# protolambda/go-kzg

Measured on AMD Instinct MI355X. Metric: KZG commitments/sec (CommitToPoly, 4096-element blob); FK20 half: value_fk20_4096, higher is better.
Workload: dtype u32; 1 GPU; CommitToPoly, 4096-coeff blobs, eth/trusted_setup.json monomial setup (s=1337), 4096 blobs/step/GPU resident in HBM, fixed-base table budget 110 GB (library default 110 GB: signed 16-bit windows, 8 of them walked by both GLV halves of every scalar, 103 GB; see table_sweep); global_batch=4096, parallelism=dp1 (independent blobs, no data-path collective)

## Files before the change

go-kzg_amd/__init__.py:

```python
import ctypes as C
import os

import numpy as np

_HERE = os.path.dirname(os.path.abspath(__file__))
LIB_PATH = os.environ.get("KZG_HIP_LIB") or os.path.join(_HERE, "libkzg_hip.so")

OK, ERR_TOO_WIDE, ERR_NOT_POW2, ERR_LEN_MISMATCH, ERR_UPPER_HALF, ERR_BAD_ARG, ERR_BAD_POINT, ERR_NO_DEVICE, ERR_HIP, ERR_UNSUPPORTED, ERR_RECOVERY, ERR_BAD_BLOB = range(12)


class KzgError(Exception):

    def __init__(self, status, msg=""):
        super().__init__("kzg_hip status %d %s" % (status, msg))
        self.status = status


class KzgPanic(KzgError):
    """The reference panics (kzg.go:22-27,44-52,74-91; fk20_single.go:60-62,140-154; bls_kilic.go:133-135)."""


class NoDeviceError(KzgError):
    pass

# ... 32 lines not shown
        "kzg_hip_points_set_table_budget_gb": (i32, [vp, C.c_double]),
        "kzg_hip_lincomb_points": (i32, [vp, vp, u64, vp]), "kzg_hip_lincomb_points_batch": (i32, [vp, vp, u64, u64, vp]),
        "kzg_hip_lincomb_points_batch_dev": (i32, [vp, vp, u64, u64, vp, vp]), "kzg_hip_g1_to_compressed": (i32, [vp, vp, u64, vp]),
        "kzg_hip_g1_from_compressed": (i32, [vp, vp, u64, vp]), "kzg_hip_g1_mul_vec": (i32, [vp, vp, vp, u64, vp]),
        "kzg_hip_generate_testing_setup_g1": (i32, [vp, vp, u64, vp]),
        "kzg_hip_g1_marshal_text": (i32, [vp, vp, u64, vp]), "kzg_hip_g1_unmarshal_text": (i32, [vp, C.c_char_p, u64, vp]),
        "kzg_hip_trusted_setup_from_json": (i32, [vp, C.c_char_p, u64, vp, vp, u64, C.POINTER(u64), C.POINTER(u64)]),
        "kzg_hip_kzg_set_table_budget_gb": (i32, [vp, C.c_double]),
        "kzg_hip_kzg_settings_new": (i32, [vp, vp, u64, pp]), "kzg_hip_kzg_settings_free": (None, [vp]),
        "kzg_hip_commit_to_poly": (i32, [vp, vp, u64, vp]), "kzg_hip_commit_to_poly_batch": (i32, [vp, vp, u64, u64, vp]),
        "kzg_hip_commit_to_poly_batch_dev": (i32, [vp, vp, u64, u64, vp, vp]),
        "kzg_hip_compute_proof_single": (i32, [vp, vp, u64, u64, vp]),
        "kzg_hip_compute_proof_single_batch": (i32, [vp, vp, u64, u64, vp, vp]),
        "kzg_hip_compute_proof_single_batch_dev": (i32, [vp, vp, u64, u64, vp, vp, vp]),
        "kzg_hip_compute_proof_multi": (i32, [vp, vp, u64, u64, u64, vp]),
        "kzg_hip_check_proof_multi_interpolation": (i32, [vp, vp, u64, vp, vp, vp]),
        "kzg_hip_g2_from_compressed": (i32, [vp, vp, u64, vp]), "kzg_hip_pairings_verify_batch": (i32, [vp, vp, vp, vp, vp, u64, vp]),
        "kzg_hip_kzg_set_secret_g2": (i32, [vp, vp, u64]), "kzg_hip_check_proof_single_batch": (i32, [vp, vp, vp, vp, vp, u64, vp]),
        "kzg_hip_check_proof_multi_batch": (i32, [vp, vp, vp, vp, vp, u64, u64, vp]),
        "kzg_hip_eth_set_setup_g2": (i32, [vp, vp, u64]), "kzg_hip_eth_verify_kzg_proof_batch": (i32, [vp, vp, vp, vp, vp, u64, vp]),
        "kzg_hip_pairing_test": (i32, [vp, vp, vp, u64, vp]),
        "kzg_hip_toeplitz_part2": (i32, [vp, vp, vp, u64, vp]), "kzg_hip_toeplitz_part3": (i32, [vp, vp, u64, vp]),
        "kzg_hip_fk20_single_settings_new": (i32, [vp, u64, pp]), "kzg_hip_fk20_single_settings_free": (None, [vp]),
        "kzg_hip_fk20_single_x_ext_fft": (i32, [vp, vp]), "kzg_hip_fk20_single": (i32, [vp, vp, u64, vp]),
        "kzg_hip_fk20_single_batch": (i32, [vp, vp, u64, u64, vp]), "kzg_hip_fk20_single_batch_dev": (i32, [vp, vp, u64, u64, vp, vp]),
        "kzg_hip_fk20_single_da_optimized": (i32, [vp, vp, u64, vp]), "kzg_hip_da_using_fk20": (i32, [vp, vp, u64, vp]),
        "kzg_hip_da_using_fk20_batch": (i32, [vp, vp, u64, u64, vp]), "kzg_hip_da_using_fk20_batch_dev": (i32, [vp, vp, u64, u64, vp, vp]),
        "kzg_hip_fk20_multi_settings_new": (i32, [vp, u64, u64, pp]), "kzg_hip_fk20_multi_settings_free": (None, [vp]),
        "kzg_hip_fk20_multi": (i32, [vp, vp, u64, vp]), "kzg_hip_fk20_multi_da_optimized": (i32, [vp, vp, u64, vp]),
        "kzg_hip_da_using_fk20_multi": (i32, [vp, vp, u64, vp]),
        "kzg_hip_da_using_fk20_multi_batch_dev": (i32, [vp, vp, u64, u64, vp, vp]),
        "kzg_hip_fk20_multi_hext_slice_dev": (i32, [vp, vp, u64, u64, u64, vp, vp]),
        "kzg_hip_fk20_multi_finish_dev": (i32, [vp, vp, i32, vp, vp]),
        "kzg_hip_eth_settings_new": (i32, [vp, vp, u64, pp]), "kzg_hip_eth_settings_free": (None, [vp]),
        "kzg_hip_eth_blob_to_kzg_commitment_batch": (i32, [vp, vp, u64, vp, vp]),
        "kzg_hip_eth_compute_kzg_proof": (i32, [vp, vp, u64, vp, vp, vp]),
        "kzg_hip_eth_compute_kzg_proof_batch": (i32, [vp, vp, u64, u64, vp, vp, vp, vp]),
        "kzg_hip_eth_compute_kzg_proof_batch_dev": (i32, [vp, vp, u64, u64, vp, vp, vp, vp, vp]),
        "kzg_hip_eth_compute_aggregate_kzg_proof": (i32, [vp, vp, u64, vp, vp]),
        "kzg_hip_eth_compute_aggregated_poly_and_commitment": (i32, [vp, vp, vp, u64, vp, vp, vp, vp]),
        "kzg_hip_test_sha256": (None, [vp, u64, vp]),
        "kzg_hip_evaluate_poly_in_evaluation_form": (i32, [vp, vp, u64, vp, u32, vp]),
        "kzg_hip_eth_evaluate_polynomial_in_evaluation_form": (i32, [vp, vp, u64, vp, vp]),
        "kzg_hip_bench_threads_fft_fr": (i32, [vp, vp, u64, u64, u32, u32, vp, C.POINTER(C.c_double)]),
        "kzg_hip_bench_drop_in_eth_proof": (i32, [vp, vp, u64, u64, u32, u32, vp, C.POINTER(C.c_double)]),
        "kzg_hip_zero_poly_via_multiplication": (i32, [vp, vp, u64, u64, vp, vp]),
        "kzg_hip_recover_poly_from_samples": (i32, [vp, vp, vp, u64, vp]),
        "kzg_hip_calibrate": (i32, [vp, C.POINTER(C.c_double), C.POINTER(C.c_double), C.POINTER(C.c_double)]),
        "kzg_hip_bench_drop_in": (i32, [vp, i32, vp, u64, u64, u32, u32, vp, C.POINTER(C.c_double)]),
        "kzg_hip_coalesce_stats": (i32, [vp, i32, C.POINTER(u64)]),
        "kzg_hip_lincomb_promotions": (i32, [vp, C.POINTER(u64), C.POINTER(u64)]),
        "kzg_hip_test_fp_inv": (i32, [vp, vp, u64, vp, vp, C.POINTER(C.c_double), C.POINTER(C.c_double)]),
        "kzg_hip_test_fr_inv": (i32, [vp, vp, u64, vp, vp, vp]),
        "kzg_hip_kzg_table_info": (i32, [vp, C.POINTER(C.c_uint32), C.POINTER(C.c_uint32), C.POINTER(u64)]), "kzg_hip_kzg_table_additions": (u32, [vp]), "kzg_hip_kzg_set_projective_outputs": (i32, [vp, i32]),
        "kzg_hip_da_using_fk20_multi_batch": (i32, [vp, vp, u64, u64, vp]),
        "kzg_hip_multi_settings_new": (i32, [C.POINTER(i32), u32, u32, vp, u64, pp]), "kzg_hip_multi_settings_free": (None, [vp]),
        "kzg_hip_multi_device_count": (u32, [vp]), "kzg_hip_multi_device": (i32, [vp, u32]),
        "kzg_hip_multi_fft": (vp, [vp, u32]), "kzg_hip_multi_kzg": (vp, [vp, u32]),
        "kzg_hip_multi_transport": (C.c_char_p, [vp]), "kzg_hip_multi_transport_note": (C.c_char_p, [vp]), "kzg_hip_multi_transport_check": (C.c_char_p, [vp]), "kzg_hip_multi_exchanges": (u64, [vp]),
        "kzg_hip_multi_set_fft_sharding": (i32, [vp, i32]), "kzg_hip_multi_set_table_budget_gb": (i32, [vp, C.c_double]),
        "kzg_hip_multi_commit_to_poly_batch": (i32, [vp, vp, u64, u64, vp]),
        "kzg_hip_multi_compute_proof_single_batch": (i32, [vp, vp, u64, u64, vp, vp]),
        "kzg_hip_multi_fft_fr_batch": (i32, [vp, vp, u64, u64, i32, vp]), "kzg_hip_multi_das_fft_extension_batch": (i32, [vp, vp, u64, u64]),
        "kzg_hip_multi_eth_settings_new": (i32, [vp, vp, u64, pp]), "kzg_hip_multi_eth_settings_free": (None, [vp]),
        "kzg_hip_multi_eth_blob_to_kzg_commitment_batch": (i32, [vp, vp, u64, vp, vp]),
        "kzg_hip_multi_eth_compute_kzg_proof_batch": (i32, [vp, vp, u64, u64, vp, vp, vp, vp]),
        "kzg_hip_multi_fk20_single_settings_new": (i32, [vp, u64, pp]), "kzg_hip_multi_fk20_single_settings_free": (None, [vp]),
        "kzg_hip_multi_da_using_fk20_batch": (i32, [vp, vp, u64, u64, vp]), "kzg_hip_multi_da_using_fk20": (i32, [vp, vp, u64, vp]),
        "kzg_hip_multi_fk20_multi_settings_new": (i32, [vp, u64, u64, pp]), "kzg_hip_multi_fk20_multi_settings_free": (None, [vp]),
        "kzg_hip_multi_da_using_fk20_multi_batch": (i32, [vp, vp, u64, u64, vp]), "kzg_hip_multi_da_using_fk20_multi": (i32, [vp, vp, u64, vp]),
        "kzg_hip_bench_poly_lincomb_dev": (i32, [vp, vp, u64, vp, u64, u64, vp, vp]),
        "kzg_hip_prof_reset": (None, [vp, i32]), "kzg_hip_prof_read": (i32, [vp, C.c_char_p, C.POINTER(C.c_double), C.POINTER(u64)]),
    }
    for name, (res, args) in sig.items():
        if os.environ.get("KZG_HIP_LIB_ALLOW_MISSING") and not hasattr(L, name):
            continue
        f = getattr(L, name)
        f.restype, f.argtypes = res, args
    _lib = L
    return L


API_SYMBOLS = None


def device_count():
    return lib().kzg_hip_device_count()


class pinned:

    def __init__(self, array):
        self.a = array

    def __enter__(self):
        _chk(lib().kzg_hip_host_register(self.a.ctypes.data, self.a.nbytes))
        return self.a

    def __exit__(self, *exc):
        lib().kzg_hip_host_unregister(self.a.ctypes.data)
        return False


_ERR_STATUS = (ERR_TOO_WIDE, ERR_NOT_POW2)


# ... 760 lines not shown
```

go-kzg_amd/csrc/capi_bench.hip:

```cpp
#include "capi_common.hpp"

namespace {
struct prof_rec { std::string name; hipEvent_t e0, e1; };
std::mutex g_prof_mu;
bool g_prof_on = false;
std::vector<prof_rec> g_prof;
}
namespace kzg {
void prof_begin(hipStream_t s, const char *name) {
    if (!g_prof_on) return;
    std::lock_guard<std::mutex> lk(g_prof_mu);
    prof_rec r; r.name = name;
    hipEventCreate(&r.e0); hipEventCreate(&r.e1);
    hipEventRecord(r.e0, s);
    g_prof.push_back(r);
}
void prof_end(hipStream_t s, const char *name) {
    if (!g_prof_on) return;
    std::lock_guard<std::mutex> lk(g_prof_mu);
    for (size_t i = g_prof.size(); i-- > 0;)
        if (g_prof[i].name == name) { hipEventRecord(g_prof[i].e1, s); break; }
}
}

// ... 130 lines not shown
            hipEventRecord(e1, s); hipEventSynchronize(e1);
            float ms = 0; hipEventElapsedTime(&ms, e0, e1);
            if (rep && ms < best) best = ms;
        }
        return (double)best * 1e-3;
    };
    const double lanes = (double)blocks * threads;
    *mad_per_s = lanes * CAL_ITERS * 8 / timed(0);
    *add_per_s = lanes * CAL_ITERS * 8 / timed(1);
    *fp_mul_per_s = lanes * 64 * 2 / timed(2);
    hipEventDestroy(e0); hipEventDestroy(e1);
    HIPCHK(hipGetLastError());
    return KZG_HIP_OK;
}
int kzg_hip_test_fp_inv(kzg_hip_fft *fs, const void *in_fp, uint64_t n, void *out_coop, void *out_lane, double *ms_coop, double *ms_lane) {
    if (!fs || !in_fp || !n || n > (1u << 20)) return KZG_HIP_ERR_BAD_ARG;
    dev_guard g(fs);
    hipStream_t s = fs->stream;
    dtmp<fp> d_in(s), d_a(s), d_b(s);
    CHK(d_in.alloc(n)); CHK(d_a.alloc(n)); CHK(d_b.alloc(n));
    HIPCHK(hipMemcpyAsync(d_in.p, in_fp, n * sizeof(fp), hipMemcpyHostToDevice, s));
    hipEvent_t e0, e1;
    HIPCHK(hipEventCreate(&e0)); HIPCHK(hipEventCreate(&e1));
    for (int which = 0; which < 2; which++) {
        void *out = which ? out_lane : out_coop; double *ms = which ? ms_lane : ms_coop;
        if (!out) continue;
        hipEventRecord(e0, s);
        launch_fp_inv_both(s, d_in.p, d_a.p, d_b.p, n, which ? 2 : 1);
        hipEventRecord(e1, s);
        HIPCHK(hipMemcpyAsync(out, which ? d_b.p : d_a.p, n * sizeof(fp), hipMemcpyDeviceToHost, s));
        HIPCHK(hipStreamSynchronize(s));
        float t = 0; hipEventElapsedTime(&t, e0, e1);
        if (ms) *ms = t;
    }
    hipEventDestroy(e0); hipEventDestroy(e1);
    HIPCHK(hipGetLastError());
    return KZG_HIP_OK;
}
int kzg_hip_test_fr_inv(kzg_hip_fft *fs, const void *in_fr, uint64_t n, void *out_coop, void *out_lane, void *out_block) {
    if (!fs || !in_fr || !n || n > (1u << 20) || !out_coop || !out_lane || !out_block) return KZG_HIP_ERR_BAD_ARG;
    dev_guard g(fs);
    hipStream_t s = fs->stream;
    dtmp<fr> d_in(s), d_a(s), d_b(s), d_c(s);
    CHK(d_in.alloc(n)); CHK(d_a.alloc(n)); CHK(d_b.alloc(n)); CHK(d_c.alloc(n));
    HIPCHK(hipMemcpyAsync(d_in.p, in_fr, n * sizeof(fr), hipMemcpyHostToDevice, s));
    launch_fr_inv_test(s, d_in.p, n, d_a.p, d_b.p, d_c.p);
    HIPCHK(hipGetLastError());
    HIPCHK(hipMemcpyAsync(out_coop, d_a.p, n * sizeof(fr), hipMemcpyDeviceToHost, s));
    HIPCHK(hipMemcpyAsync(out_lane, d_b.p, n * sizeof(fr), hipMemcpyDeviceToHost, s));
    HIPCHK(hipMemcpyAsync(out_block, d_c.p, n * sizeof(fr), hipMemcpyDeviceToHost, s));
    HIPCHK(hipStreamSynchronize(s));
    return KZG_HIP_OK;
}
int kzg_hip_coalesce_stats(kzg_hip_kzg *ks, int op, uint64_t out[8]) {
    if (!ks || !out || op < 0 || op > 1) return KZG_HIP_ERR_BAD_ARG;
    for (int i = 0; i < 8; i++) out[i] = 0;
    std::lock_guard<std::mutex> lk(ks->fs->mu);
    coalescer *co = op == 0 ? ks->co_commit.get() : ks->co_proof.get();
    if (co) co->stats(out);
    return KZG_HIP_OK;
}
void kzg_hip_prof_reset(kzg_hip_fft *fs, int enable) {
    (void)fs;
    std::lock_guard<std::mutex> lk(g_prof_mu);
    for (auto &r : g_prof) { hipEventDestroy(r.e0); hipEventDestroy(r.e1); }
    g_prof.clear();
    g_prof_on = enable != 0;
}
int kzg_hip_prof_read(kzg_hip_fft *fs, const char *kernel, double *total_ms, uint64_t *launches) {
    if (!fs || !kernel) return KZG_HIP_ERR_BAD_ARG;
    std::lock_guard<std::mutex> lk(g_prof_mu);
    double tot = 0; uint64_t cnt = 0;
    for (auto &r : g_prof) {
        if (r.name != kernel) continue;
        HIPCHK(hipEventSynchronize(r.e1));
        float ms = 0;
        HIPCHK(hipEventElapsedTime(&ms, r.e0, r.e1));
        tot += ms; cnt++;
    }
    if (total_ms) *total_ms = tot;
    if (launches) *launches = cnt;
    return KZG_HIP_OK;
}
```

go-kzg_amd/csrc/capi_kzg.hip:

```cpp
#include "capi_common.hpp"

int kzg_settings_build(kzg_hip_fft *fs, const void *points_g1, uint64_t n, kzg_hip_kzg **out) {
    dev_guard g(fs);
    hipStream_t s = fs->stream;
    std::unique_ptr<kzg_hip_kzg, void (*)(kzg_hip_kzg *)> own(new kzg_hip_kzg, kzg_hip_kzg_settings_free);
    kzg_hip_kzg *ks = own.get();
    ks->fs = fs; ks->n_setup = n;
    dtmp<g1j> d_raw(s);
    CHK(d_raw.alloc(n));
    HIPCHK(hipMalloc((void **)&ks->d_secret, n * sizeof(g1j)));
    HIPCHK(hipMalloc((void **)&ks->d_secret_a, n * sizeof(g1a)));
    HIPCHK(hipMemcpyAsync(d_raw.p, points_g1, n * sizeof(g1j), hipMemcpyHostToDevice, s));
    launch_g1_from_kilic(s, d_raw.p, n);
    launch_g1_normalize(s, d_raw.p, ks->d_secret, n);
    launch_g1_to_affine(s, ks->d_secret, ks->d_secret_a, n);
    HIPCHK(hipGetLastError());
    HIPCHK(hipStreamSynchronize(s));
    *out = own.release();
    return KZG_HIP_OK;
}
int kzg_hip_kzg_settings_new(kzg_hip_fft *fs, const void *secret_g1, uint64_t n_setup, kzg_hip_kzg **out) {
    if (!fs || !out || !secret_g1) return KZG_HIP_ERR_BAD_ARG;
    *out = nullptr;
    if (n_setup < fs->W) return KZG_HIP_ERR_LEN_MISMATCH;
// ... 15 lines not shown
double table_budget_gb(const char *env, double cap_gb, double headroom_gb) {
    if (const char *e = getenv(env)) return atof(e);
    size_t free_b = 0, total_b = 0;
    if (hipMemGetInfo(&free_b, &total_b) != hipSuccess) return 0.0;
    double g = (double)free_b / 1e9 - headroom_gb;
    return g > cap_gb ? cap_gb : (g > 0.0 ? g : 0.0);
}
uint32_t fb_windows(uint32_t c) {
    uint32_t nw = (255 + c - 1) / c, sh = c * (nw - 1);
    uint64_t top = (0x73eda753299d7d48ull >> (sh - 192)) + 1;
    return top > (1ull << (c - 1)) ? nw + 1 : nw;
}

#ifndef FB_DEFAULT_BUDGET_GB
#define FB_DEFAULT_BUDGET_GB 110.0
#endif
uint32_t fb_windows_glv(uint32_t c) { return (128 + c - 1) / c; }
bool fb_glv_enabled() {
    static const bool on = [] { const char *e = getenv("KZG_HIP_FB_GLV"); return !(e && !strcmp(e, "0")); }();
    return on;
}
int ensure_fixed_table(kzg_hip_kzg *ks, hipStream_t) {
    if (ks->d_fixed || ks->fixed_plan.c == 0xffffffffu) return KZG_HIP_OK;
    hipStream_t s = ks->fs->stream;
    double budget_gb = ks->budget_gb >= 0.0 ? ks->budget_gb : table_budget_gb("KZG_HIP_FB_BUDGET_GB", FB_DEFAULT_BUDGET_GB, 24.0);
    if (ks->n_setup < 64) { ks->fixed_plan.c = 0xffffffffu; return KZG_HIP_OK; }
    const bool glv = fb_glv_enabled();
    for (uint32_t c = 16; c >= 5; c--) {
        if (glv ? (c == 14) : (c == 15)) continue;
        const uint32_t nwin = glv ? fb_windows_glv(c) : fb_windows(c);
        double bytes = (double)nwin * (double)ks->n_setup * (double)(1u << (c - 1)) * sizeof(g1a);
        if (bytes > budget_gb * 1e9) continue;
        msm_plan p{};
        p.c = c; p.nwin = nwin; p.nb = 1u << (c - 1); p.ngroups = 1; p.fixed = 1; p.glv = glv ? 1 : 0; p.table_n = ks->n_setup;
        size_t entries = (size_t)p.nwin * ks->n_setup * p.nb;
        g1a *tab = nullptr;
        if (hipMalloc((void **)&tab, entries * sizeof(g1a)) != hipSuccess) { (void)hipGetLastError(); continue; }
        hipError_t e = launch_fb_build(s, ks->d_secret_a, ks->n_setup, p.c, p.nwin, tab);
        if (e == hipSuccess) e = hipStreamSynchronize(s);
        if (e != hipSuccess) { (void)hipGetLastError(); hipFree(tab); continue; }
        ks->d_fixed = tab; ks->fixed_plan = p;
        return KZG_HIP_OK;
    }
    ks->fixed_plan.c = 0xffffffffu;
    return KZG_HIP_OK;
}

int commit_rows(kzg_hip_kzg *ks, hipStream_t s, const fr *d_sc, uint64_t n, uint64_t batch, g1j *d_out, uint64_t sc_stride, bool to_kilic) {
    CHK(ensure_fixed_table(ks, s));
    bool fixed = ks->d_fixed != nullptr;
    if (!sc_stride) sc_stride = n;
    msm_plan p = fixed ? ks->fixed_plan : classic_plan(ks->n_setup);
    if (!fixed && !msm_index_range_ok(p, n)) return KZG_HIP_ERR_TOO_WIDE;
    size_t ws_main = fixed ? fb_partials_bytes(n, batch) : msm_workspace_bytes(p, n, batch);
    dtmp<uint8_t> d_ws(s);
    CHK(d_ws.alloc(ws_main));
    if (fixed) launch_fb_msm(s, ks->d_fixed, p.table_n, p.c, p.nwin, d_sc, sc_stride, n, batch, d_ws.p, d_out, to_kilic, p.glv != 0, to_kilic && ks->projective.load(std::memory_order_relaxed));
    else launch_msm(s, p, ks->d_secret_a, d_sc, sc_stride, n, batch, d_ws.p, d_out, to_kilic);
    HIPCHK(hipGetLastError());
    return KZG_HIP_OK;
}
int kzg_hip_kzg_set_table_budget_gb(kzg_hip_kzg *ks, double gb) {
    if (!ks || !(gb >= 0.0)) return KZG_HIP_ERR_BAD_ARG;
    std::unique_lock<std::shared_mutex> tl(ks->tab_mu);
    dev_guard g(ks->fs);
    if (ks->d_fixed) { HIPCHK(hipDeviceSynchronize()); HIPCHK(hipFree(ks->d_fixed)); ks->d_fixed = nullptr; }
    ks->fixed_plan = msm_plan{};
    ks->budget_gb = gb;
    return KZG_HIP_OK;
}

int kzg_hip_commit_to_poly_batch_dev(kzg_hip_kzg *ks, const void *d_coeffs_fr, uint64_t n, uint64_t batch, void *d_out_g1, void *stream) {
    if (!ks || !d_out_g1) return KZG_HIP_ERR_BAD_ARG;
    if (n > ks->n_setup) return KZG_HIP_ERR_LEN_MISMATCH;
    if (!batch) return KZG_HIP_OK;
    if (n == 0 || !d_coeffs_fr) return KZG_HIP_ERR_BAD_ARG;
    dev_guard g(ks->fs);
    return commit_rows(ks, (hipStream_t)stream, (const fr *)d_coeffs_fr, n, batch, (g1j *)d_out_g1);
}
namespace {
std::mutex g_reg_mu;
std::map<uintptr_t, size_t> g_registered;
}
const void *host_mapped_pointer(const void *host, size_t bytes) {
    hipPointerAttribute_t a;
    if (hipPointerGetAttributes(&a, host) != hipSuccess) { (void)hipGetLastError(); return nullptr; }
    if (a.type != hipMemoryTypeHost || !a.devicePointer) return nullptr;
    const uintptr_t h = (uintptr_t)host;
    {
        std::lock_guard<std::mutex> lk(g_reg_mu);
        auto it = g_registered.upper_bound(h);
        if (it != g_registered.begin()) {
            --it;
            if (h >= it->first && h < it->first + it->second) return (h + bytes <= it->first + it->second) ? a.devicePointer : nullptr;
        }
    }
    hipDeviceptr_t base = nullptr; size_t size = 0;
    if (hipMemGetAddressRange(&base, &size, (hipDeviceptr_t)a.devicePointer) != hipSuccess) { (void)hipGetLastError(); return nullptr; }
    const uintptr_t d = (uintptr_t)a.devicePointer, b = (uintptr_t)base;
    return (d >= b && d + bytes <= b + size) ? a.devicePointer : nullptr;
}
int h2d_copy(void *dst, const void *src, size_t bytes, hipStream_t s) {
    uintptr_t p = (uintptr_t)src; uint8_t *d = (uint8_t *)dst;
    while (bytes) {
        size_t chunk = bytes;
        {
            std::lock_guard<std::mutex> lk(g_reg_mu);
// ... 339 lines not shown
```

go-kzg_amd/csrc/internal.hpp:

```cpp
#pragma once
#include <hip/hip_runtime.h>
#include <stdint.h>
#include "field.hpp"
#include "g1.hpp"

namespace kzg {

void launch_fr_fft(hipStream_t s, const fr *in, uint64_t in_stride, uint64_t n_in, fr *out, uint64_t n, uint64_t batch,
                   const fr *roots, uint64_t W, const fr *scale, const uint32_t *tw4096 = nullptr, const fr *roots_l = nullptr);
void launch_das_ext(hipStream_t s, fr *vals, uint64_t n, uint64_t batch, const fr *expanded, const fr *reversed, uint64_t W,
                    const fr *inv_n, const uint32_t *tw2048 = nullptr);
void launch_toeplitz_coeffs(hipStream_t s, const fr *poly, uint64_t poly_stride, uint64_t n, uint64_t l, uint64_t batch, fr *out,
                            const fr *scale);
void launch_quotient_linear(hipStream_t s, const fr *poly, uint64_t poly_stride, uint64_t n, uint64_t batch, const fr *x, fr *q, uint64_t q_stride);
void launch_fr_from_u64(hipStream_t s, const uint64_t *in, uint64_t in_stride, fr *out, uint64_t n);
void launch_fr_zero_tails(hipStream_t s, fr *rows, uint64_t n_max, uint64_t batch, const uint64_t *lens, uint64_t lens_stride);
void launch_fr_any_nonzero(hipStream_t s, const fr *vals, uint64_t n, uint32_t *flag);
void launch_fr_powers(hipStream_t s, const fr *base, uint64_t n, fr *out);

void launch_fr_from_le32(hipStream_t s, const uint8_t *in, fr *out, uint64_t per_blob, uint64_t batch, uint32_t *bad);
void launch_fr_to_le32(hipStream_t s, const fr *in, uint8_t *out, uint64_t n);
void launch_fr_bitrev_gather(hipStream_t s, const fr *in, fr *out, uint64_t n);
constexpr uint64_t ZERO_TREE_LEAF = 16;
void launch_zero_leaves(hipStream_t s, const fr *expanded, uint64_t stride, const uint64_t *missing, uint64_t n_missing, uint64_t leaves, fr *a);
// ... 5 lines not shown
void launch_eth_quotient(hipStream_t s, const fr *poly, uint64_t poly_stride, const fr *domain, uint64_t n, uint64_t batch, const fr *z, uint64_t z_stride,
                         const fr *inv_n, fr *q, fr *y_out, uint32_t *flag, uint64_t dom_stride = 1, fr *scratch = nullptr);
uint64_t eth_quotient_scratch_elems(uint64_t n, uint64_t batch);

void launch_fr_scale_by_inv_powers(hipStream_t s, fr *c, const fr *x, uint64_t n, fr *xpow_n);

void launch_zero_eval_direct(hipStream_t s, const fr *expanded, uint64_t stride, const uint64_t *missing, uint64_t n_missing, uint64_t length, fr *zero_eval);
void launch_fr_scale_by_powers(hipStream_t s, fr *poly, const fr *base, uint64_t n);
void launch_fr_pointwise(hipStream_t s, const fr *a, const fr *b, const uint8_t *present, fr *out, uint64_t n, int mode, uint32_t *flag);

void launch_g1_mul_vec(hipStream_t s, const g1j *pts, uint64_t pts_mod, const fr *scalars, uint64_t s_stride, uint64_t n, g1j *out);
hipError_t launch_g1_file_msm(hipStream_t s, const g1j *files, const fr *scalars, uint64_t nfiles, uint64_t k2, uint64_t j0, uint64_t cnt,
                              uint64_t batch, g1j *out);
void launch_g1_bitrev_copy(hipStream_t s, const g1j *in, uint64_t in_stride, uint64_t n_valid, g1j *out, uint64_t n, uint64_t batch);
void launch_g1_fft_stage(hipStream_t s, g1j *data, uint64_t n, uint64_t batch, uint64_t m, const fr *roots, const int8_t *wnaf, uint64_t W);
void launch_g1_fft_stage_dif(hipStream_t s, g1j *data, uint64_t n, uint64_t batch, uint64_t m, const fr *roots, const int8_t *wnaf, uint64_t W);
void launch_g1_clear_odd(hipStream_t s, g1j *data, uint64_t n_total);
void launch_g1_take_even(hipStream_t s, const g1j *in, g1j *out, uint64_t total);
bool g1_quad_enabled();
void launch_fb_direct_pass1(hipStream_t s, const g1a *table, uint64_t table_n, uint32_t c, uint32_t nwin, const fr *scalars, const fr *roots, uint64_t W, uint64_t batch,
                            uint32_t logR, g1j *out, bool glv = false);
void launch_g1_stage_coop_dif(hipStream_t s, int lanes, g1j *data, uint64_t n, uint64_t batch, uint64_t m, const fr *roots, const int8_t *wnaf, uint64_t W, uint64_t total);
void launch_g1_stage_coop_dit(hipStream_t s, int lanes, g1j *data, uint64_t n, uint64_t batch, uint64_t m, const fr *roots, const int8_t *wnaf, uint64_t W, uint64_t total);
void launch_g1_direct_coop(hipStream_t s, int lanes, uint32_t wgs, size_t pad_lds, const g1j *src, uint64_t src_stride, uint64_t src_valid, g1j *dst, uint32_t logn, uint32_t logR,
                           uint64_t Ns, const fr *roots, uint64_t W, const fr *sc, uint64_t total, uint32_t logT, uint32_t logU);
void launch_g1_fft_direct(hipStream_t s, const g1j *in, uint64_t in_stride, uint64_t n_valid, g1j *data, g1j *tmp, uint64_t n, uint64_t batch, const fr *roots,
                          uint64_t W, const fr *scale, uint32_t max_logr = 4, int lanes = 1, uint32_t bits_done = 0, uint64_t n_out = 0);
void launch_g1_normalize(hipStream_t s, const g1j *in, g1j *out, uint64_t n, bool to_kilic = false);
void launch_fr_inv_test(hipStream_t s, const fr *in, uint64_t n, fr *out_coop, fr *out_lane, fr *out_block);
void launch_fp_inv_both(hipStream_t s, const fp *in, fp *out_coop, fp *out_lane, uint64_t n, int mode);
void launch_g1_from_kilic(hipStream_t s, g1j *data, uint64_t n);
void launch_g1_to_affine(hipStream_t s, const g1j *in, g1a *out, uint64_t n);
void launch_g1_compress(hipStream_t s, const g1j *in, uint8_t *out48, uint64_t n);
void launch_g1_decompress(hipStream_t s, const uint8_t *in48, g1j *out, uint64_t n, uint32_t *bad_flag);
void launch_g1_fixed_base_powers(hipStream_t s, const fr *powers, uint64_t n, g1j *out);

uint64_t device_simd_lanes();
inline uint64_t device_simds() { return device_simd_lanes() / 64; }
struct msm_plan {
    uint32_t c;
    uint32_t nwin;
    uint32_t nb;
    uint32_t ngroups;
    uint32_t fixed;
    uint32_t glv;
    uint64_t table_n;
};
inline bool msm_index_range_ok(const msm_plan &p, uint64_t n) { return n < (1ull << 27) && 2 * p.table_n < (1ull << 30); }
size_t msm_workspace_bytes(const msm_plan &p, uint64_t n, uint64_t batch);
void launch_msm(hipStream_t s, const msm_plan &p, const g1a *table, const fr *scalars, uint64_t sc_stride, uint64_t n, uint64_t batch, void *workspace, g1j *out,
                bool to_kilic);
void launch_msm_window_table(hipStream_t s, const g1a *pts, uint64_t n, uint32_t c, uint32_t nwin, g1j *tmp, g1a *out);

size_t fb_partials_bytes(uint64_t n, uint64_t batch);
hipError_t launch_fb_build(hipStream_t s, const g1a *pts, uint64_t n, uint32_t c, uint32_t nwin, g1a *table);
void launch_fb_msm(hipStream_t s, const g1a *table, uint64_t table_n, uint32_t c, uint32_t nwin, const fr *scalars, uint64_t sc_stride, uint64_t n,
                   uint64_t batch, void *partials, g1j *out, bool to_kilic, bool glv = false, bool projective = false);

void launch_fb_mul_vec(hipStream_t s, const g1a *table, uint64_t table_n, uint32_t c, uint32_t nwin, const fr *scalars, uint64_t row, uint64_t j0,
                       uint64_t cnt, uint64_t batch, g1j *out, bool glv = false);
void launch_fb_mul_vec_dif2(hipStream_t s, const g1a *table, uint64_t table_n, uint32_t c, uint32_t nwin, const fr *scalars, const fr *roots, uint64_t W,
                            uint64_t batch, g1j *out, bool glv = false);
void launch_fb_mul_vec_files(hipStream_t s, const g1a *table, uint64_t table_n, uint32_t c, uint32_t nwin, const fr *scalars, uint64_t row, uint64_t j0,
                             uint64_t cnt, uint64_t batch, g1j *out, bool glv = false);
void launch_g1_sum_files(hipStream_t s, const g1j *tmp, uint64_t nfiles, uint64_t cnt, uint64_t batch, g1j *out);

struct g2j; struct g2_prepared;
void launch_g2_from_compressed(hipStream_t s, const uint8_t *in96, g2j *out_kilic, uint64_t n, uint32_t *bad_flag);
void launch_g2_prepare(hipStream_t s, const g2j *in_kilic, uint64_t n, g2_prepared *out);
void launch_pairs_g1_from_kilic(hipStream_t s, const g1j *a1, const g1j *b1, uint64_t n, g1j *p0, g1j *p1);
void launch_kzg_check_inputs(hipStream_t s, const g1j *c, const g1j *pi, const fr *ys, const g1j *es, const fr *bs, uint64_t n, g1j *p0, g1j *p1);
void launch_fr_rows_scale_by_inv_powers(hipStream_t s, fr *c, uint64_t np, const fr *xs, uint64_t count, fr *xpow_n);
void launch_eth_check_inputs(hipStream_t s, const uint8_t *c48, const uint8_t *zs, const uint8_t *ys, const uint8_t *pi48, uint64_t n, g1j *p0, g1j *p1, uint8_t *status);
void launch_pairing_check(hipStream_t s, bool shared_lines, const g2_prepared *q0, const g2_prepared *q1, const g1j *p0, const g1j *p1, uint64_t n, uint8_t *ok);
void launch_pairing_value(hipStream_t s, const g1j *g1_kilic, const g2_prepared *q, uint64_t n, fp *out);

void prof_begin(hipStream_t s, const char *name);
void prof_end(hipStream_t s, const char *name);

}
```

go-kzg_amd/csrc/k_msm.hip:

```cpp
#include "internal.hpp"
#include "g1_quad.hpp"
#include "coop_inv.hpp"
#include <atomic>
#include <cstring>

namespace kzg {

#define MSM_SORT_T 1024
#define MSM_ACC_BLOCK 128
#define MSM_NB 128

struct fb_partial { uint32_t w[52]; uint32_t inf; };
__device__ __forceinline__ void fb_partial_store(fb_partial &o, const g1x_acc &a) {
#pragma unroll
    for (int i = 0; i < 13; i++) { o.w[i] = a.v.x.l[i]; o.w[13 + i] = a.v.y.l[i]; o.w[26 + i] = a.v.zz.l[i]; o.w[39 + i] = a.v.zzz.l[i]; }
    o.inf = a.inf ? 1u : 0u;
}
__device__ __forceinline__ void fb_partial_load(const fb_partial &p, g1xq &v) {
#pragma unroll
    for (int i = 0; i < 13; i++) { v.x.l[i] = p.w[i]; v.y.l[i] = p.w[13 + i]; v.zz.l[i] = p.w[26 + i]; v.zzz.l[i] = p.w[39 + i]; }
}

template <uint32_t DELTA, bool ROW> __device__ __forceinline__ uint32_t lane_down(uint32_t v) {
    if constexpr (ROW && DELTA < 16) return (uint32_t)__builtin_amdgcn_update_dpp((int)v, (int)v, 0x100 + DELTA, 0xf, 0xf, false);
// ... 728 lines not shown
        if (in_phi && !phi) { if (!acc.inf) acc.v.x = mulq(acc.v.x, unpackq(glv_beta())); in_phi = false; }
        uint32_t m[4], sgn;
        if (keep_ok && !phi) {
            const uint32_t at = slot < FB_KEEP ? slot : 0; slot++;
#pragma unroll
            for (int j = 0; j < 4; j++) m[j] = kept[at][j];
            sgn = kept[at][4];
            if (slot == (uint32_t)(nvh / L)) slot = 0;
        } else {
            const glv_halves h = glv_split_signed(from_mont<FrP>(sc[i]));
#pragma unroll
            for (int j = 0; j < 4; j++) m[j] = phi ? h.k2[j] : h.k1[j];
            sgn = phi ? h.neg2 : h.neg1;
            if (keep_ok) {
                const uint32_t at = slot < FB_KEEP ? slot : 0; slot++;
#pragma unroll
                for (int j = 0; j < 4; j++) kept[at][j] = h.k1[j];
                kept[at][4] = h.neg1;
                if (slot == (uint32_t)(nvh / L)) slot = 0;
            }
        }
        uint32_t raw, carry = 0, mag, ng;
        if (SPLIT) {
#pragma nounroll
            for (uint32_t w = 0; w < w0; w++) carry = (mag_bits(m, w * c, c) + carry > D) ? 1u : 0u;
        }
        raw = mag_bits(m, w0 * c, c) + carry;
        if (raw > D) { carry = 1; mag = (1u << c) - raw; ng = 1; } else { carry = 0; mag = raw; ng = 0; }
        g1a qn = table[((uint64_t)w0 * table_n + i) * D + (mag ? mag - 1 : 0)];
#pragma nounroll
        for (uint32_t w = w0; w < w1; w++) {
            g1a q = qn;
            const uint32_t cmag = mag, cng = ng;
            if (w + 1 < w1) {
                raw = mag_bits(m, (w + 1) * c, c) + carry;
                if (raw > D) { carry = 1; mag = (1u << c) - raw; ng = 1; } else { carry = 0; mag = raw; ng = 0; }
                qn = table[((uint64_t)(w + 1) * table_n + i) * D + (mag ? mag - 1 : 0)];
            }
            if (cmag) {
                if (cng ^ sgn) q.y = neg<FpP>(q.y);
                acc.add(q);
                in_phi = phi;
            }
        }
    }
    if (in_phi && !acc.inf) acc.v.x = mulq(acc.v.x, unpackq(glv_beta()));
#ifdef KZG_REDUCE_WAVE_COOP
    fb_block_reduce_coop(acc, buf, &lds, tid);
#else
    fb_block_reduce_quad(acc, buf, tid);
#endif
    if (tid == 0) fb_partial_store(partials[blockIdx.x], acc);
}
__global__ __launch_bounds__(256) void k_fb_finish(const fb_partial *partials, uint32_t blocks_per_blob, uint64_t batch, g1j *out, int to_kilic) {
    __shared__ fb_partial buf[64];
    const uint64_t b = blockIdx.x;
#ifdef KZG_REDUCE_WAVE_COOP
    __shared__ coop_lds lds;
    coop_ctx c; c.L = &lds; c.wave = threadIdx.x >> 6; c.col = threadIdx.x & 63u; c.set = 0;
    const uint32_t col = c.col;
    g1x_acc acc; acc.init();
    acc.v = g1xq_from_affine(g1a_inf());
    const uint32_t rounds = (blocks_per_blob + 63) / 64;
#pragma nounroll
    for (uint32_t r = 0; r < rounds; r++) {
        const uint32_t j = r * 64 + col;
        const bool have = j < blocks_per_blob;
        const fb_partial &pj = partials[b * blocks_per_blob + (have ? j : 0)];
        g1xq w; fb_partial_load(pj, w);
        coop_acc_add(acc, w, !have || pj.inf != 0, c);
    }
    const uint32_t live = blocks_per_blob < 64 ? blocks_per_blob : 64;
    uint32_t off = 1;
    while (off < live) off *= 2;
#pragma nounroll
    for (off >>= 1; off >= 1; off >>= 1) {
        const bool have = col < off && col + off < live;
        g1xq w; uint32_t wi;
        point_down_any(w, wi, acc.v, acc.inf ? 1u : 0u, off);
        coop_acc_add(acc, w, !have || wi != 0, c);
    }
    const bool first_wave = c.wave == 0;
#else
    const uint32_t tid = threadIdx.x, role = tid & 3u, quad = tid >> 2, col = tid & 63u;
#ifdef KZG_FINISH_TIMING
    const uint64_t tf0 = wall_clock64();
#endif
    g1x_acc acc; acc.init();
    acc.v = g1xq_from_affine(g1a_inf());
    const uint32_t rounds = (blocks_per_blob + 63) / 64;
    g1xq wn; bool wn_inf;
    { const bool have = quad < blocks_per_blob; const fb_partial &pj = partials[b * blocks_per_blob + (have ? quad : 0)]; fb_partial_load(pj, wn); wn_inf = !have || pj.inf != 0; }
#pragma nounroll
    for (uint32_t r = 0; r < rounds; r++) {
        const g1xq w = wn; const bool winf = wn_inf;
        if (r + 1 < rounds) {
            const uint32_t j = (r + 1) * 64 + quad;
            const bool have = j < blocks_per_blob;
            const fb_partial &pj = partials[b * blocks_per_blob + (have ? j : 0)];
            fb_partial_load(pj, wn); wn_inf = !have || pj.inf != 0;
        }
        quad_acc_add_nl(acc, w, winf, role);
    }
#ifdef KZG_FINISH_TIMING
    __syncthreads(); const uint64_t tf1 = wall_clock64();
#endif
// ... 228 lines not shown
    out[t] = acc.to_jac();
}
void launch_fb_mul_vec_files(hipStream_t s, const g1a *table, uint64_t table_n, uint32_t c, uint32_t nwin, const fr *scalars, uint64_t row, uint64_t j0,
                             uint64_t cnt, uint64_t batch, g1j *out, bool glv) {
    uint64_t total = batch * cnt;
    if (!total) return;
    prof_begin(s, "fb_mul_vec");
    if (glv) hipLaunchKernelGGL(k_fb_mul_vec_files<true>, dim3((uint32_t)((total + FB_BLOCK - 1) / FB_BLOCK)), dim3(FB_BLOCK), 0, s, table, table_n, c, nwin, 1u << (c - 1), scalars,
                                j0, cnt, row, total, out);
    else hipLaunchKernelGGL(k_fb_mul_vec_files<false>, dim3((uint32_t)((total + FB_BLOCK - 1) / FB_BLOCK)), dim3(FB_BLOCK), 0, s, table, table_n, c, nwin, 1u << (c - 1), scalars,
                            j0, cnt, row, total, out);
    prof_end(s, "fb_mul_vec");
}
void launch_fb_mul_vec(hipStream_t s, const g1a *table, uint64_t table_n, uint32_t c, uint32_t nwin, const fr *scalars, uint64_t row, uint64_t j0,
                       uint64_t cnt, uint64_t batch, g1j *out, bool glv) {
    uint64_t total = batch * (table_n / row) * cnt;
    if (!total) return;
    prof_begin(s, "fb_mul_vec");
    if (glv) hipLaunchKernelGGL(k_fb_mul_vec<true>, dim3((uint32_t)((total + FB_BLOCK - 1) / FB_BLOCK)), dim3(FB_BLOCK), 0, s, table, table_n, c, nwin, 1u << (c - 1), scalars,
                                j0, cnt, row, total, out);
    else hipLaunchKernelGGL(k_fb_mul_vec<false>, dim3((uint32_t)((total + FB_BLOCK - 1) / FB_BLOCK)), dim3(FB_BLOCK), 0, s, table, table_n, c, nwin, 1u << (c - 1), scalars,
                            j0, cnt, row, total, out);
    prof_end(s, "fb_mul_vec");
}

uint64_t device_simd_lanes() {
    static std::atomic<uint64_t> lanes_of_device[64];
    int dev = 0;
    (void)hipGetDevice(&dev);
    std::atomic<uint64_t> &slot = lanes_of_device[dev >= 0 && dev < 64 ? dev : 0];
    uint64_t lanes = slot.load(std::memory_order_relaxed);
    if (!lanes) {
        int cus = 256;
        if (hipDeviceGetAttribute(&cus, hipDeviceAttributeMultiprocessorCount, dev) != hipSuccess) { (void)hipGetLastError(); cus = 256; }
        lanes = (uint64_t)(cus > 0 ? cus : 256) * 4 * 64;
        slot.store(lanes, std::memory_order_relaxed);
    }
    return lanes;
}
static uint32_t fb_blocks_per_blob(uint64_t n, uint64_t batch, uint32_t *wsplit = nullptr) {
    static const uint64_t forced_lanes = [] { const char *e = getenv("KZG_HIP_FB_LANES"); return e ? strtoull(e, nullptr, 10) : 0ull; }();
    uint64_t lanes = forced_lanes ? forced_lanes : 2 * device_simd_lanes();
    if (lanes < FB_ACC_BLOCK) lanes = FB_ACC_BLOCK;
    uint64_t target = lanes / FB_ACC_BLOCK;
    uint64_t bpb = target / (batch ? batch : 1);
    uint32_t split = 1;
    while (split < 8 && (batch ? batch : 1) * n * split * 2 <= lanes) split *= 2;
    if (wsplit) *wsplit = split;
    uint64_t maxb = (n * split + FB_ACC_BLOCK - 1) / FB_ACC_BLOCK;
    if (bpb > maxb) bpb = maxb;
    if (bpb < 1) bpb = 1;
    return (uint32_t)bpb;
}
size_t fb_partials_bytes(uint64_t n, uint64_t batch) { return (((size_t)std::max(fb_blocks_per_blob(n, batch), fb_blocks_per_blob(2 * n, batch)) * batch * sizeof(fb_partial)) + 15) / 16 * 16; }

void launch_fb_msm(hipStream_t s, const g1a *table, uint64_t table_n, uint32_t c, uint32_t nwin, const fr *scalars, uint64_t sc_stride, uint64_t n,
                   uint64_t batch, void *partials, g1j *out, bool to_kilic, bool glv, bool projective) {
    if (!batch) return;
    const int fin = (to_kilic ? 1 : 0) | (projective ? 2 : 0);
    uint32_t split = 1;
    uint32_t bpb = fb_blocks_per_blob(glv ? 2 * n : n, batch, &split);
    if (split > nwin) split = nwin;
    prof_begin(s, "fb_accumulate");
    if (glv) {
        if (split > 1) hipLaunchKernelGGL(k_fb_accumulate_glv<true>, dim3((uint32_t)(batch * bpb)), dim3(FB_ACC_BLOCK), 0, s, table, table_n, c, nwin, 1u << (c - 1), scalars, sc_stride, n,
                                          bpb, split, (fb_partial *)partials);
        else hipLaunchKernelGGL(k_fb_accumulate_glv<false>, dim3((uint32_t)(batch * bpb)), dim3(FB_ACC_BLOCK), 0, s, table, table_n, c, nwin, 1u << (c - 1), scalars, sc_stride, n, bpb,
                                1u, (fb_partial *)partials);
    } else if (split > 1) hipLaunchKernelGGL(k_fb_accumulate<true>, dim3((uint32_t)(batch * bpb)), dim3(FB_ACC_BLOCK), 0, s, table, table_n, c, nwin, 1u << (c - 1), scalars, sc_stride, n,
                                      bpb, split, (fb_partial *)partials);
    else hipLaunchKernelGGL(k_fb_accumulate<false>, dim3((uint32_t)(batch * bpb)), dim3(FB_ACC_BLOCK), 0, s, table, table_n, c, nwin, 1u << (c - 1), scalars, sc_stride, n, bpb,
                            1u, (fb_partial *)partials);
    prof_end(s, "fb_accumulate");
    if (bpb <= FB_FINISH_LANES_MAX) hipLaunchKernelGGL(k_fb_finish_lanes, dim3((uint32_t)((batch + 63) / 64)), dim3(64), 0, s, (const fb_partial *)partials, bpb, batch, out, fin);
    else hipLaunchKernelGGL(k_fb_finish, dim3((uint32_t)batch), dim3(256), 0, s, (const fb_partial *)partials, bpb, batch, out, fin);
}
hipError_t launch_fb_build(hipStream_t s, const g1a *pts, uint64_t n, uint32_t c, uint32_t nwin, g1a *table) {
    uint32_t D = 1u << (c - 1);
    g1j *rows_j = nullptr; g1a *rows = nullptr; fp *ztmp = nullptr, *ptmp = nullptr;
    uint64_t lanes_all = (uint64_t)nwin * n;
    hipError_t e;
    if ((e = hipMallocAsync((void **)&rows_j, lanes_all * sizeof(g1j), s)) != hipSuccess) return e;
    if ((e = hipMallocAsync((void **)&rows, lanes_all * sizeof(g1a), s)) != hipSuccess) { hipFreeAsync(rows_j, s); return e; }
    launch_msm_window_table(s, pts, n, c, nwin, rows_j, rows);
    uint64_t per_win = n * D * sizeof(fp);
    uint32_t slab = (uint32_t)((1ull << 30) / (per_win ? per_win : 1));
    if (slab < 1) slab = 1;
    if (slab > nwin) slab = nwin;
    if ((e = hipMallocAsync((void **)&ztmp, (uint64_t)slab * per_win, s)) != hipSuccess) { hipFreeAsync(rows_j, s); hipFreeAsync(rows, s); return e; }
    if ((e = hipMallocAsync((void **)&ptmp, (uint64_t)slab * per_win, s)) != hipSuccess) { hipFreeAsync(rows_j, s); hipFreeAsync(rows, s); hipFreeAsync(ztmp, s); return e; }
    for (uint32_t w0 = 0; w0 < nwin; w0 += slab) {
        uint32_t ws = (w0 + slab <= nwin) ? slab : nwin - w0;
        uint64_t lanes = (uint64_t)ws * n;
        uint32_t S = D;
        while (S > 64 && lanes * (D / S) < (1ull << 20)) S >>= 1;
        dim3 g((uint32_t)((lanes * (D / S) + FB_BLOCK - 1) / FB_BLOCK)), b(FB_BLOCK);
        hipLaunchKernelGGL(k_fb_build_pass1, g, b, 0, s, rows + (uint64_t)w0 * n, lanes, D, S, table + (uint64_t)w0 * n * D, ztmp);
        hipLaunchKernelGGL(k_fb_build_pass2, g, b, 0, s, lanes, D, S, table + (uint64_t)w0 * n * D, ztmp, ptmp);
    }
    hipFreeAsync(rows_j, s); hipFreeAsync(rows, s); hipFreeAsync(ztmp, s); hipFreeAsync(ptmp, s);
    return hipGetLastError();
}

__global__ __launch_bounds__(MSM_ACC_BLOCK, 2) void k_msm_window_rows(const g1a *pts, uint64_t n, uint32_t c, uint32_t nwin, g1j *tmp) {
    uint64_t i = blockIdx.x * (uint64_t)blockDim.x + threadIdx.x;
    if (i >= n) return;
    g1j q = to_jac(pts[i]);
#pragma nounroll
    for (uint32_t w = 0; w < nwin; w++) {
        tmp[(uint64_t)w * n + i] = q;
#pragma nounroll
        for (uint32_t j = 0; j < c; j++) q = g1_dbl(q);
    }
}
void launch_msm_window_table(hipStream_t s, const g1a *pts, uint64_t n, uint32_t c, uint32_t nwin, g1j *tmp, g1a *out) {
    if (!n) return;
    hipLaunchKernelGGL(k_msm_window_rows, dim3((uint32_t)((n + MSM_ACC_BLOCK - 1) / MSM_ACC_BLOCK)), dim3(MSM_ACC_BLOCK), 0, s, pts, n, c, nwin, tmp);
// ... 5 lines not shown
```

go-kzg_amd/csrc/kzg_hip_internal.h:

```cpp
#ifndef KZG_HIP_INTERNAL_H
#define KZG_HIP_INTERNAL_H
#include "../../include/kzg_hip.h"
#ifdef __cplusplus
extern "C" {
#endif
#pragma GCC visibility push(default)

void kzg_hip_prof_reset(kzg_hip_fft *fs, int enable);
int kzg_hip_prof_read(kzg_hip_fft *fs, const char *kernel, double *total_ms, uint64_t *launches);
int kzg_hip_calibrate(kzg_hip_fft *fs, double *mad_per_s, double *add_per_s, double *fp_mul_per_s);
int kzg_hip_bench_drop_in(kzg_hip_kzg *ks, int op, const void *blobs_fr, uint64_t n, uint64_t nblobs, unsigned threads, unsigned calls, void *out_g1,
                          double *seconds);
int kzg_hip_bench_drop_in_eth_proof(kzg_hip_eth *eth, const void *polys_fr, uint64_t n, uint64_t npolys, unsigned threads, unsigned calls, void *out48,
                                    double *seconds);
int kzg_hip_bench_threads_fft_fr(kzg_hip_fft *fs, const void *vals_fr, uint64_t n, uint64_t nrows, unsigned threads, unsigned calls, void *out_fr, double *seconds);
int kzg_hip_bench_poly_lincomb_dev(kzg_hip_fft *fs, const void *d_vectors_fr, uint64_t stride, const void *d_scalars_fr, uint64_t count, uint64_t n, void *d_out_fr,
                                   void *stream);
int kzg_hip_coalesce_stats(kzg_hip_kzg *ks, int op, uint64_t out[8]);
int kzg_hip_test_fp_inv(kzg_hip_fft *fs, const void *in_fp, uint64_t n, void *out_coop, void *out_lane, double *ms_coop, double *ms_lane);
int kzg_hip_lincomb_promotions(kzg_hip_fft *fs, uint64_t *promoted, uint64_t *served);
int kzg_hip_test_fr_inv(kzg_hip_fft *fs, const void *in_fr, uint64_t n, void *out_coop, void *out_lane, void *out_block);
void kzg_hip_test_sha256(const void *data, uint64_t len, void *out32);

int kzg_hip_pairing_test(kzg_hip_fft *fs, const void *g1, const void *g2, uint64_t n, void *out_fp12);

#pragma GCC visibility pop
#ifdef __cplusplus
}
#endif
#endif
```

Before: 95900 commitments/s.

## Precompute signed GLV window digits in a separate pass before fixed-base walk

Adds a kernel that GLV-splits each scalar once and writes signed 16-bit window codes plus sign bits to a workspace buffer. A new walk kernel reads those codes and software-pipelines the table gathers one window ahead, instead of decoding digits inline in the accumulate loop. The goal is to take scalar decomposition and carry logic off the latency-bound gather loop and overlap the next table load with the current point addition. The cost is an extra kernel launch and a digits buffer of batch*n*2*nwin uint16 written and read back through HBM. The new path is on by default when GLV is used and the accumulation is not split across windows.

```diff
diff --git a/go-kzg_amd/__init__.py b/go-kzg_amd/__init__.py
--- a/go-kzg_amd/__init__.py
+++ b/go-kzg_amd/__init__.py
@@ -108,6 +108,7 @@
         "kzg_hip_lincomb_promotions": (i32, [vp, C.POINTER(u64), C.POINTER(u64)]),
         "kzg_hip_test_fp_inv": (i32, [vp, vp, u64, vp, vp, C.POINTER(C.c_double), C.POINTER(C.c_double)]),
         "kzg_hip_test_fr_inv": (i32, [vp, vp, u64, vp, vp, vp]),
+        "kzg_hip_test_fb_digits": (i32, [vp, vp, u64, u32, vp, vp]),
         "kzg_hip_kzg_table_info": (i32, [vp, C.POINTER(C.c_uint32), C.POINTER(C.c_uint32), C.POINTER(u64)]), "kzg_hip_kzg_table_additions": (u32, [vp]), "kzg_hip_kzg_set_projective_outputs": (i32, [vp, i32]),
         "kzg_hip_da_using_fk20_multi_batch": (i32, [vp, vp, u64, u64, vp]),
         "kzg_hip_multi_settings_new": (i32, [C.POINTER(i32), u32, u32, vp, u64, pp]), "kzg_hip_multi_settings_free": (None, [vp]),
diff --git a/go-kzg_amd/csrc/capi_bench.hip b/go-kzg_amd/csrc/capi_bench.hip
--- a/go-kzg_amd/csrc/capi_bench.hip
+++ b/go-kzg_amd/csrc/capi_bench.hip
@@ -206,6 +206,21 @@
     HIPCHK(hipStreamSynchronize(s));
     return KZG_HIP_OK;
 }
+int kzg_hip_test_fb_digits(kzg_hip_fft *fs, const void *in_fr, uint64_t n, uint32_t c, void *out_codes, void *out_signs) {
+    if (!fs || !in_fr || !n || n > (1u << 20) || c < 2 || c > 16 || !out_codes || !out_signs) return KZG_HIP_ERR_BAD_ARG;
+    dev_guard g(fs);
+    hipStream_t s = fs->stream;
+    const uint32_t nwin = fb_windows_glv(c);
+    dtmp<fr> d_in(s); dtmp<uint16_t> d_dig(s); dtmp<uint8_t> d_sg(s);
+    CHK(d_in.alloc(n)); CHK(d_dig.alloc((size_t)2 * nwin * n)); CHK(d_sg.alloc(n));
+    HIPCHK(hipMemcpyAsync(d_in.p, in_fr, n * sizeof(fr), hipMemcpyHostToDevice, s));
+    launch_fb_digits_glv(s, d_in.p, n, n, 1, c, nwin, d_dig.p, d_sg.p);
+    HIPCHK(hipGetLastError());
+    HIPCHK(hipMemcpyAsync(out_codes, d_dig.p, (size_t)2 * nwin * n * sizeof(uint16_t), hipMemcpyDeviceToHost, s));
+    HIPCHK(hipMemcpyAsync(out_signs, d_sg.p, n, hipMemcpyDeviceToHost, s));
+    HIPCHK(hipStreamSynchronize(s));
+    return KZG_HIP_OK;
+}
 int kzg_hip_coalesce_stats(kzg_hip_kzg *ks, int op, uint64_t out[8]) {
     if (!ks || !out || op < 0 || op > 1) return KZG_HIP_ERR_BAD_ARG;
     for (int i = 0; i < 8; i++) out[i] = 0;
diff --git a/go-kzg_amd/csrc/capi_kzg.hip b/go-kzg_amd/csrc/capi_kzg.hip
--- a/go-kzg_amd/csrc/capi_kzg.hip
+++ b/go-kzg_amd/csrc/capi_kzg.hip
@@ -91,7 +91,7 @@
     if (!sc_stride) sc_stride = n;
     msm_plan p = fixed ? ks->fixed_plan : classic_plan(ks->n_setup);
     if (!fixed && !msm_index_range_ok(p, n)) return KZG_HIP_ERR_TOO_WIDE;
-    size_t ws_main = fixed ? fb_partials_bytes(n, batch) : msm_workspace_bytes(p, n, batch);
+    size_t ws_main = fixed ? fb_workspace_bytes(n, batch, p.nwin, p.glv != 0) : msm_workspace_bytes(p, n, batch);
     dtmp<uint8_t> d_ws(s);
     CHK(d_ws.alloc(ws_main));
     if (fixed) launch_fb_msm(s, ks->d_fixed, p.table_n, p.c, p.nwin, d_sc, sc_stride, n, batch, d_ws.p, d_out, to_kilic, p.glv != 0, to_kilic && ks->projective.load(std::memory_order_relaxed));
diff --git a/go-kzg_amd/csrc/internal.hpp b/go-kzg_amd/csrc/internal.hpp
--- a/go-kzg_amd/csrc/internal.hpp
+++ b/go-kzg_amd/csrc/internal.hpp
@@ -81,10 +81,11 @@
                 bool to_kilic);
 void launch_msm_window_table(hipStream_t s, const g1a *pts, uint64_t n, uint32_t c, uint32_t nwin, g1j *tmp, g1a *out);
 
-size_t fb_partials_bytes(uint64_t n, uint64_t batch);
+size_t fb_workspace_bytes(uint64_t n, uint64_t batch, uint32_t nwin, bool glv);
+void launch_fb_digits_glv(hipStream_t s, const fr *scalars, uint64_t sc_stride, uint64_t n, uint64_t batch, uint32_t c, uint32_t nwin, uint16_t *dig, uint8_t *sg);
 hipError_t launch_fb_build(hipStream_t s, const g1a *pts, uint64_t n, uint32_t c, uint32_t nwin, g1a *table);
 void launch_fb_msm(hipStream_t s, const g1a *table, uint64_t table_n, uint32_t c, uint32_t nwin, const fr *scalars, uint64_t sc_stride, uint64_t n,
-                   uint64_t batch, void *partials, g1j *out, bool to_kilic, bool glv = false, bool projective = false);
+                   uint64_t batch, void *workspace, g1j *out, bool to_kilic, bool glv = false, bool projective = false);
 
 void launch_fb_mul_vec(hipStream_t s, const g1a *table, uint64_t table_n, uint32_t c, uint32_t nwin, const fr *scalars, uint64_t row, uint64_t j0,
                        uint64_t cnt, uint64_t batch, g1j *out, bool glv = false);
diff --git a/go-kzg_amd/csrc/k_msm.hip b/go-kzg_amd/csrc/k_msm.hip
--- a/go-kzg_amd/csrc/k_msm.hip
+++ b/go-kzg_amd/csrc/k_msm.hip
@@ -804,6 +804,70 @@
 #endif
     if (tid == 0) fb_partial_store(partials[blockIdx.x], acc);
 }
+
+#define FB_DIGIT_ZERO 0xffffu
+static size_t fb_digits_bytes(uint64_t n, uint64_t batch, uint32_t nwin) { return ((size_t)batch * n * 2 * nwin * sizeof(uint16_t) + 255) / 256 * 256 + ((size_t)batch * n + 255) / 256 * 256; }
+__global__ __launch_bounds__(256) void k_fb_digits_glv(const fr *scalars, uint64_t sc_stride, uint64_t n, uint64_t batch, uint32_t c, uint32_t nwin, uint32_t D,
+                                                       uint16_t *dig, uint8_t *sg) {
+    const uint64_t t = blockIdx.x * (uint64_t)blockDim.x + threadIdx.x;
+    if (t >= n * batch) return;
+    const uint64_t b = t / n, i = t - b * n;
+    const glv_halves h = glv_split_signed(from_mont<FrP>(scalars[b * sc_stride + i]));
+#pragma unroll
+    for (uint32_t half = 0; half < 2; half++) {
+        const uint32_t (&m)[4] = half ? h.k1 : h.k2;
+        uint16_t *row = dig + (b * 2 + half) * nwin * n + i;
+        uint32_t carry = 0;
+#pragma nounroll
+        for (uint32_t w = 0; w < nwin; w++) {
+            const uint32_t raw = mag_bits(m, w * c, c) + carry;
+            uint32_t mag, ng;
+            if (raw > D) { carry = 1; mag = (1u << c) - raw; ng = 1; } else { carry = 0; mag = raw; ng = 0; }
+            row[(uint64_t)w * n] = (uint16_t)(mag ? (mag - 1) | (ng << 15) : FB_DIGIT_ZERO);
+        }
+    }
+    sg[t] = (uint8_t)(h.neg2 | (h.neg1 << 1));
+}
+template <uint32_t WAVES> __global__ __launch_bounds__(FB_ACC_BLOCK, WAVES) void k_fb_walk_digits(const g1a *table, uint64_t table_n, uint32_t nwin, uint32_t D,
+                                                                                               const uint16_t *dig, const uint8_t *sg, uint64_t n,
+                                                                                               uint32_t blocks_per_blob, fb_partial *partials) {
+    __shared__ fb_partial buf[64];
+    const uint32_t tid = threadIdx.x;
+    const uint64_t blob = blockIdx.x / blocks_per_blob; const uint32_t blk = blockIdx.x % blocks_per_blob;
+    const uint64_t L = (uint64_t)blocks_per_blob * FB_ACC_BLOCK;
+    const uint64_t wstride = table_n * D;
+    g1x_acc acc; acc.init();
+    bool in_phi = false;
+    for (uint64_t v = (uint64_t)blk * FB_ACC_BLOCK + tid; v < 2 * n; v += L) {
+        const bool phi = v < n;
+        const uint64_t i = phi ? v : v - n;
+        if (in_phi && !phi) { if (!acc.inf) acc.v.x = mulq(acc.v.x, unpackq(glv_beta())); in_phi = false; }
+        const uint16_t *row = dig + (blob * 2 + (phi ? 0u : 1u)) * nwin * n + i;
+        const uint32_t sgn = ((uint32_t)sg[blob * n + i] >> (phi ? 0 : 1)) & 1u;
+        const g1a *tw = table + i * D;
+        uint32_t code = row[0];
+        uint32_t cnext = nwin > 1 ? (uint32_t)row[n] : FB_DIGIT_ZERO;
+        g1a qn = tw[code == FB_DIGIT_ZERO ? 0u : code & 0x7fffu];
+#pragma nounroll
+        for (uint32_t w = 0; w < nwin; w++) {
+            g1a q = qn;
+            const uint32_t cc = code;
+            if (w + 1 < nwin) {
+                code = cnext;
+                if (w + 2 < nwin) cnext = row[(uint64_t)(w + 2) * n];
+                qn = tw[(uint64_t)(w + 1) * wstride + (code == FB_DIGIT_ZERO ? 0u : code & 0x7fffu)];
+            }
+            if (cc != FB_DIGIT_ZERO) {
+                if ((cc >> 15) ^ sgn) q.y = neg<FpP>(q.y);
+                acc.add(q);
+                in_phi = phi;
+            }
+        }
+    }
+    if (in_phi && !acc.inf) acc.v.x = mulq(acc.v.x, unpackq(glv_beta()));
+    fb_block_reduce_quad(acc, buf, tid);
+    if (tid == 0) fb_partial_store(partials[blockIdx.x], acc);
+}
 __global__ __launch_bounds__(256) void k_fb_finish(const fb_partial *partials, uint32_t blocks_per_blob, uint64_t batch, g1j *out, int to_kilic) {
     __shared__ fb_partial buf[64];
     const uint64_t b = blockIdx.x;
@@ -1138,17 +1202,39 @@
     if (bpb < 1) bpb = 1;
     return (uint32_t)bpb;
 }
-size_t fb_partials_bytes(uint64_t n, uint64_t batch) { return (((size_t)std::max(fb_blocks_per_blob(n, batch), fb_blocks_per_blob(2 * n, batch)) * batch * sizeof(fb_partial)) + 15) / 16 * 16; }
-
+static size_t fb_partials_bytes(uint64_t n, uint64_t batch) { return (((size_t)std::max(fb_blocks_per_blob(n, batch), fb_blocks_per_blob(2 * n, batch)) * batch * sizeof(fb_partial)) + 15) / 16 * 16; }
+static bool fb_digit_walk(uint64_t n, uint64_t batch, uint32_t nwin, bool glv) {
+    static const bool on = [] { const char *e = getenv("KZG_HIP_FB_DIGITS"); return !(e && !strcmp(e, "0")); }();
+    if (!on || !glv) return false;
+    uint32_t split = 1;
+    fb_blocks_per_blob(2 * n, batch, &split);
+    return split <= 1 || nwin <= 1;
+}
+size_t fb_workspace_bytes(uint64_t n, uint64_t batch, uint32_t nwin, bool glv) {
+    const size_t pb = fb_partials_bytes(n, batch);
+    return fb_digit_walk(n, batch, nwin, glv) ? (pb + 255) / 256 * 256 + fb_digits_bytes(n, batch, nwin) : pb;
+}
+
+void launch_fb_digits_glv(hipStream_t s, const fr *scalars, uint64_t sc_stride, uint64_t n, uint64_t batch, uint32_t c, uint32_t nwin, uint16_t *dig, uint8_t *sg) {
+    if (!n || !batch) return;
+    hipLaunchKernelGGL(k_fb_digits_glv, dim3((uint32_t)((batch * n + 255) / 256)), dim3(256), 0, s, scalars, sc_stride, n, batch, c, nwin, 1u << (c - 1), dig, sg);
+}
 void launch_fb_msm(hipStream_t s, const g1a *table, uint64_t table_n, uint32_t c, uint32_t nwin, const fr *scalars, uint64_t sc_stride, uint64_t n,
-                   uint64_t batch, void *partials, g1j *out, bool to_kilic, bool glv, bool projective) {
+                   uint64_t batch, void *workspace, g1j *out, bool to_kilic, bool glv, bool projective) {
     if (!batch) return;
     const int fin = (to_kilic ? 1 : 0) | (projective ? 2 : 0);
     uint32_t split = 1;
     uint32_t bpb = fb_blocks_per_blob(glv ? 2 * n : n, batch, &split);
     if (split > nwin) split = nwin;
+    void *partials = workspace;
     prof_begin(s, "fb_accumulate");
-    if (glv) {
+    if (fb_digit_walk(n, batch, nwin, glv)) {
+        uint16_t *dig = (uint16_t *)((uint8_t *)workspace + (fb_partials_bytes(n, batch) + 255) / 256 * 256);
+        uint8_t *sg = (uint8_t *)dig + ((size_t)batch * n * 2 * nwin * sizeof(uint16_t) + 255) / 256 * 256;
+        launch_fb_digits_glv(s, scalars, sc_stride, n, batch, c, nwin, dig, sg);
+        hipLaunchKernelGGL(k_fb_walk_digits<FB_ACC_WAVES>, dim3((uint32_t)(batch * bpb)), dim3(FB_ACC_BLOCK), 0, s, table, table_n, nwin, 1u << (c - 1),
+                           (const uint16_t *)dig, (const uint8_t *)sg, n, bpb, (fb_partial *)partials);
+    } else if (glv) {
         if (split > 1) hipLaunchKernelGGL(k_fb_accumulate_glv<true>, dim3((uint32_t)(batch * bpb)), dim3(FB_ACC_BLOCK), 0, s, table, table_n, c, nwin, 1u << (c - 1), scalars, sc_stride, n,
                                           bpb, split, (fb_partial *)partials);
         else hipLaunchKernelGGL(k_fb_accumulate_glv<false>, dim3((uint32_t)(batch * bpb)), dim3(FB_ACC_BLOCK), 0, s, table, table_n, c, nwin, 1u << (c - 1), scalars, sc_stride, n, bpb,
diff --git a/go-kzg_amd/csrc/kzg_hip_internal.h b/go-kzg_amd/csrc/kzg_hip_internal.h
--- a/go-kzg_amd/csrc/kzg_hip_internal.h
+++ b/go-kzg_amd/csrc/kzg_hip_internal.h
@@ -20,6 +20,7 @@
 int kzg_hip_test_fp_inv(kzg_hip_fft *fs, const void *in_fp, uint64_t n, void *out_coop, void *out_lane, double *ms_coop, double *ms_lane);
 int kzg_hip_lincomb_promotions(kzg_hip_fft *fs, uint64_t *promoted, uint64_t *served);
 int kzg_hip_test_fr_inv(kzg_hip_fft *fs, const void *in_fr, uint64_t n, void *out_coop, void *out_lane, void *out_block);
+int kzg_hip_test_fb_digits(kzg_hip_fft *fs, const void *in_fr, uint64_t n, uint32_t c, void *out_codes, void *out_signs);
 void kzg_hip_test_sha256(const void *data, uint64_t len, void *out32);
 
 int kzg_hip_pairing_test(kzg_hip_fft *fs, const void *g1, const void *g2, uint64_t n, void *out_fp12);
```

After: 95980 commitments/s (median of 4 runs). No clear change (+0.1%).
